# maelaubert/VulkanSift

Hardware: AMD Instinct MI355X
Metric: SIFT detect+match frames/sec (640x480, ~2k kp) (higher is better)
Workload: dtype f32

## Files before the change

include/vksift_hip.h:

```cpp
#ifndef VKSIFT_HIP_H
#define VKSIFT_HIP_H

#include <stddef.h>
#include <stdint.h>

#ifdef __cplusplus
extern "C"
{
#endif

#define VKSIFT_HIP_MAX_TAPS 20
#define VKSIFT_HIP_MATCH_CHUNKS 32
#define VKSIFT_HIP_MATCH_SMALL_NA 1536u
#define VKSIFT_HIP_MATCH_SMALL_NB 4096u
#define VKSIFT_HIP_MATCH_SCRATCH_U32(na, nb) (2u * (size_t)(na) + (size_t)(nb) + 72u + (size_t)(na) * 16u * VKSIFT_HIP_MATCH_CHUNKS)
#define VKSIFT_HIP_ABI_VERSION 6u
#define VKSIFT_HIP_GATHER_SLOTS 512u
#define VKSIFT_HIP_MATCH_SLOTS 256u
#define VKSIFT_HIP_MATCH_PK_NB 32768u
#define VKSIFT_HIP_MAX_ORI 18
#define VKSIFT_HIP_MAX_OCTAVE_SIDE 16383u

  typedef void *vksift_hip_stream;
  typedef void *vksift_hip_graph;
// ... 22 lines not shown
  int vksift_hip_event_sync(vksift_hip_event e);
  int vksift_hip_event_busy(vksift_hip_event e);
  float vksift_hip_event_elapsed_ms(vksift_hip_event a, vksift_hip_event b);
  int vksift_hip_stream_wait_event(vksift_hip_stream s, vksift_hip_event e);
  int vksift_hip_capture_begin(vksift_hip_stream s);
  int vksift_hip_capture_end(vksift_hip_stream s, vksift_hip_graph *out);
  int vksift_hip_graph_launch(vksift_hip_graph g, vksift_hip_stream s);
  void vksift_hip_graph_destroy(vksift_hip_graph g);
  int vksift_hip_memcpy_h2d(void *dst, const void *src, size_t n, vksift_hip_stream s);
  int vksift_hip_memcpy_d2h(void *dst, const void *src, size_t n, vksift_hip_stream s);
  int vksift_hip_memcpy_d2d(void *dst, const void *src, size_t n, vksift_hip_stream s);
  int vksift_hip_memcpy2d_d2h(void *dst, size_t dpitch, const void *src, size_t spitch, size_t width_bytes, size_t height, vksift_hip_stream s);
  int vksift_hip_post_words(uint32_t *host_mapped_dst, const uint32_t *src, size_t n_words, vksift_hip_stream s);
  int vksift_hip_memset(void *dst, int value, size_t n, vksift_hip_stream s);
  const char *vksift_hip_error_string(int err);
  void vksift_hip_range_push(const char *name);
  void vksift_hip_range_pop(void);

  enum
  {
    VKSIFT_TUNE_WG_TARGET = 0,
    VKSIFT_TUNE_WIDE_MASK = 1,
    VKSIFT_TUNE_MULTI_MAX = 2,
    VKSIFT_TUNE_REFINE_PTR = 3,
    VKSIFT_TUNE_SCAN_FORM = 4,
    VKSIFT_TUNE_PAIR_FORM = 5,
    VKSIFT_TUNE_PYR_GATE = 6,
    VKSIFT_TUNE_DENSE_ROWS = 7,
    VKSIFT_TUNE_SEED_WG = 8,
    VKSIFT_TUNE_SCAN_BAND = 9,
    VKSIFT_TUNE_TAIL_MULTI = 10,
    VKSIFT_TUNE_ZERO_COPY = 11,
    VKSIFT_TUNE_MIN_MARCH = 12,
    VKSIFT_TUNE_COUNT = 16
  };
  int vksift_hip_tune(int knob, int value);
  int vksift_hip_tune_get(int knob);


  typedef struct
  {
    float *base;
    uint32_t w, h;
    uint32_t pitch;
    uint64_t img_stride;
    uint32_t fp16;
    uint32_t reverse;
  } vksift_hip_Plane;

  int vksift_hip_input_blit(const uint8_t *src, uint32_t sw, uint32_t sh, uint64_t src_img_stride, vksift_hip_Plane dst, uint32_t batch,
                            vksift_hip_stream s);

  int vksift_hip_blur(vksift_hip_Plane src, vksift_hip_Plane dst, const float *taps, uint32_t ntaps, uint32_t batch, vksift_hip_stream s);

  int vksift_hip_blur_pair(vksift_hip_Plane src, vksift_hip_Plane dst1, vksift_hip_Plane dst2, const float *taps1, uint32_t ntaps1, const float *taps2,
                           uint32_t ntaps2, uint32_t batch, vksift_hip_stream s);

  int vksift_hip_blur_form(vksift_hip_Plane src, vksift_hip_Plane dst, uint32_t ntaps, uint32_t batch);

  int vksift_hip_blur_multi(const vksift_hip_Plane *src, const vksift_hip_Plane *dst, uint32_t n, const float *taps, uint32_t ntaps, uint32_t batch,
                            vksift_hip_stream s);

  int vksift_hip_blur_downsample(vksift_hip_Plane src, vksift_hip_Plane dst, vksift_hip_Plane next, const float *taps, uint32_t ntaps, uint32_t batch,
                                 vksift_hip_stream s);

  int vksift_hip_seed_upsampled(const uint8_t *src, uint32_t sw, uint32_t sh, uint64_t src_img_stride, vksift_hip_Plane dst, const float *taps, uint32_t ntaps,
// ... 133 lines not shown
```

vulkansift_amd/build.py:

```python
import hashlib
import os
import subprocess
import sys

PKG = os.path.dirname(os.path.abspath(__file__))
ROOT = os.path.dirname(PKG)
CSRC = os.path.join(PKG, "csrc")
OUT_DIR = os.path.join(PKG, "lib")
OBJ_DIR = os.path.join(OUT_DIR, "obj")
LIB_PATH = os.path.join(OUT_DIR, "libvulkansift.so")

HOST_SRCS = ["host/vksift_api.c", "host/vksift_instance.c", "host/vksift_mem.c", "host/vksift_detect.c", "host/vksift_stage.c", "host/vksift_defer.c", "host/vksift_buffers.c", "host/vksift_match.c", "host/vksift_verify.c", "host/vksift_refine.c", "host/vksift_guided.c",
             "host/vksift_ext.c", "host/vksift_sharded.c", "host/vksift_hostmath.c", "host/vksift_log.c", "host/vksift_synth.c"]
HIP_SRCS = ["hip/runtime.hip", "hip/pyramid.hip", "hip/extrema.hip", "hip/features.hip", "hip/match.hip", "hip/records.hip", "hip/verify.hip", "hip/refine.hip", "hip/refine_f.hip", "hip/guided.hip"]

ROCM = os.environ.get("ROCM_PATH", "/opt/rocm")
HIPCC = os.path.join(ROCM, "bin", "hipcc")
INCLUDES = ["-I" + os.path.join(ROOT, "include"), "-I" + os.path.join(CSRC, "host"), "-I" + CSRC]

CFLAGS = ["-O2", "-std=gnu11", "-fPIC", "-fexceptions", "-ffp-contract=off", "-fno-fast-math", "-mavx2", "-mfma", "-Wall", "-Wextra",
          "-Wno-unused-parameter"]
HIPFLAGS = ["--offload-arch=gfx950", "-O3", "-std=c++17", "-fPIC", "-ffp-contract=off", "-fno-fast-math", "-Wall", "-Wno-unused-function",
            "-fno-gpu-rdc"]


def _newer(target, deps):
    if not os.path.exists(target):
        return True
    t = os.path.getmtime(target)
    return any(os.path.getmtime(d) > t for d in deps if os.path.exists(d))


_TOOL_VERSION = {}


def _tool_version(tool):
    if tool not in _TOOL_VERSION:
        r = subprocess.run([tool, "--version"], capture_output=True, text=True)
        _TOOL_VERSION[tool] = (r.stdout + r.stderr).strip()
    return _TOOL_VERSION[tool]


def _signature(cmd, src, headers):
    h = hashlib.sha256()
    h.update(("\0".join(cmd).replace(ROOT, "<root>") + "\0" + _tool_version(cmd[0])).encode())
    for path in [src] + sorted(headers):
        h.update(os.path.relpath(path, ROOT).encode() + b"\0")
# ... 97 lines not shown
```

vulkansift_amd/csrc/hip/extrema.hip:

```cpp
#include <hip/hip_runtime.h>
#include <type_traits>
#include <vector>
#include <stdint.h>
#include <stdlib.h>

#include "../detmath.h"
#include "multi.h"
#include "records.h"
#include "vksift_hip.h"

namespace
{

struct DogView
{
  const float *base;
  int w, h, pitch;
  size_t plane;
  int S;
};

template <bool F16>
__device__ __forceinline__ float ld(const DogView &d, int s, int x, int y)
{
  if (s < 0 || s > d.S + 1)
    return 0.f;
  if (F16)
  {
    const _Float16 *p = (const _Float16 *)d.base + (size_t)s * d.plane + (size_t)y * d.pitch + x;
    return (float)(_Float16)((float)p[d.plane] - (float)p[0]);
  }
  const float *p = d.base + (size_t)s * d.plane + (size_t)y * d.pitch + x;
  return p[d.plane] - p[0];
}

struct KpRecord
{
  float x, y, scale_x, scale_y;
  uint32_t scale_idx;
  int32_t octave_idx;
  float sigma, orientation, intensity;
};

struct Dog19
{
  float c;
  float sp, sm, xp, xm, yp, ym;
  float sp_xp, sp_xm, sm_xp, sm_xm;
  float sp_yp, sp_ym, sm_yp, sm_ym;
  float xp_yp, xp_ym, xm_yp, xm_ym;
};

template <bool F16>
struct PtrLoader
{
  static constexpr int UNROLL_STEPS = 1;
  const DogView &d;
  __device__ __forceinline__ Dog19 operator()(int x, int y, int s) const
  {
    Dog19 v;
    v.c = ld<F16>(d, s, x, y);
    v.sp = ld<F16>(d, s + 1, x, y), v.sm = ld<F16>(d, s - 1, x, y);
    v.xp = ld<F16>(d, s, x + 1, y), v.xm = ld<F16>(d, s, x - 1, y);
    v.yp = ld<F16>(d, s, x, y + 1), v.ym = ld<F16>(d, s, x, y - 1);
    v.sp_xp = ld<F16>(d, s + 1, x + 1, y), v.sp_xm = ld<F16>(d, s + 1, x - 1, y), v.sm_xp = ld<F16>(d, s - 1, x + 1, y), v.sm_xm = ld<F16>(d, s - 1, x - 1, y);
    v.sp_yp = ld<F16>(d, s + 1, x, y + 1), v.sp_ym = ld<F16>(d, s + 1, x, y - 1), v.sm_yp = ld<F16>(d, s - 1, x, y + 1), v.sm_ym = ld<F16>(d, s - 1, x, y - 1);
    v.xp_yp = ld<F16>(d, s, x + 1, y + 1), v.xp_ym = ld<F16>(d, s, x + 1, y - 1), v.xm_yp = ld<F16>(d, s, x - 1, y + 1), v.xm_ym = ld<F16>(d, s, x - 1, y - 1);
    return v;
  }
};

template <bool F16>
struct BufLoader
{
  static constexpr int UNROLL_STEPS = 5;
  static constexpr unsigned EB = F16 ? 2u : 4u;
  const __amdgpu_buffer_rsrc_t rsrc;
  const int pitch;
  const unsigned plane;
  const int S;
  __device__ __forceinline__ float tex(unsigned base, int row_off) const
  {
    if (F16)
      return (float)__builtin_bit_cast(_Float16, (unsigned short)__builtin_amdgcn_raw_buffer_load_b16(rsrc, base, row_off, 0));
    return __uint_as_float(__builtin_amdgcn_raw_buffer_load_b32(rsrc, base, row_off, 0));
  }
  static __device__ __forceinline__ float dog(float hi, float lo) { return F16 ? (float)(_Float16)(hi - lo) : hi - lo; }
  __device__ __forceinline__ Dog19 operator()(int x, int y, int s) const
  {
    const int pitch_b = pitch * (int)EB;
    const unsigned plane_b = plane * EB;
    const unsigned b0 = ((unsigned)s * plane + (unsigned)(y - 1) * (unsigned)pitch + (unsigned)(x - 1)) * EB;
    const unsigned bm = b0 - plane_b, b1 = b0 + plane_b, b2 = b1 + plane_b;
    float g0[3][3], g1[3][3];
#pragma unroll
    for (int j = 0; j < 3; j++)
#pragma unroll
      for (int i = 0; i < 3; i++)
      {
        g0[j][i] = tex(b0 + (unsigned)i * EB, j * pitch_b);
        g1[j][i] = tex(b1 + (unsigned)i * EB, j * pitch_b);
      }
    const float gm_c = tex(bm + EB, pitch_b), gm_xm = tex(bm, pitch_b), gm_xp = tex(bm + 2u * EB, pitch_b), gm_ym = tex(bm + EB, 0), gm_yp = tex(bm + EB, 2 * pitch_b);
    const float g2_c = tex(b2 + EB, pitch_b), g2_xm = tex(b2, pitch_b), g2_xp = tex(b2 + 2u * EB, pitch_b), g2_ym = tex(b2 + EB, 0), g2_yp = tex(b2 + EB, 2 * pitch_b);
    const bool up = s + 1 <= S + 1;
    Dog19 v;
    v.sp = up ? dog(g2_c, g1[1][1]) : 0.f, v.sm = dog(g0[1][1], gm_c);
    v.sp_xp = up ? dog(g2_xp, g1[1][2]) : 0.f, v.sp_xm = up ? dog(g2_xm, g1[1][0]) : 0.f;
    v.sp_yp = up ? dog(g2_yp, g1[2][1]) : 0.f, v.sp_ym = up ? dog(g2_ym, g1[0][1]) : 0.f;
    v.sm_xp = dog(g0[1][2], gm_xp), v.sm_xm = dog(g0[1][0], gm_xm), v.sm_yp = dog(g0[2][1], gm_yp), v.sm_ym = dog(g0[0][1], gm_ym);
    float d0[3][3];
#pragma unroll
    for (int j = 0; j < 3; j++)
#pragma unroll
      for (int i = 0; i < 3; i++)
        d0[j][i] = dog(g1[j][i], g0[j][i]);
    v.c = d0[1][1];
    v.xp = d0[1][2], v.xm = d0[1][0], v.yp = d0[2][1], v.ym = d0[0][1];
    v.xp_yp = d0[2][2], v.xp_ym = d0[0][2], v.xm_yp = d0[2][0], v.xm_ym = d0[0][0];
    return v;
  }
};

template <class Load>
__device__ bool refine_core(const Load &load, int W, int H, int S, int x, int y, int s, float dog_threshold, float edge_limit, float seed_sigma, int octave_idx,
                            KpRecord *kp)
{
  float oX = 0.f, oY = 0.f, oS = 0.f, gX = 0.f, gY = 0.f, gS = 0.f;
  float vc = 0.f, xp = 0.f, xm = 0.f, yp = 0.f, ym = 0.f, h23 = 0.f;
  int rx = x, ry = y, rs = s;
#pragma unroll Load::UNROLL_STEPS
  for (int step = 0; step < 5; step++)
  {
    const Dog19 v = load(rx, ry, rs);
    vc = v.c;
    xp = v.xp, xm = v.xm, yp = v.yp, ym = v.ym;
    gS = 0.5f * (v.sp - v.sm);
    gX = 0.5f * (xp - xm);
    gY = 0.5f * (yp - ym);
    float h11 = v.sp + v.sm - 2.f * vc;
    float h22 = xp + xm - 2.f * vc;
    float h33 = yp + ym - 2.f * vc;
    float h12 = 0.25f * (v.sp_xp - v.sp_xm - v.sm_xp + v.sm_xm);
    float h13 = 0.25f * (v.sp_yp - v.sp_ym - v.sm_yp + v.sm_ym);
    h23 = 0.25f * (v.xp_yp - v.xp_ym - v.xm_yp + v.xm_ym);

    float det = h11 * ((h22 * h33) - (h23 * h23)) - h12 * ((h12 * h33) - (h13 * h23)) + h13 * ((h12 * h23) - (h13 * h22));
    if (det == 0.0f)
      return false;
    float i11 = ((h22 * h33) - (h23 * h23)) / det;
    float i12 = -1.f * ((h12 * h33) - (h13 * h23)) / det;
    float i13 = ((h12 * h23) - (h13 * h22)) / det;
    float i22 = ((h11 * h33) - (h13 * h13)) / det;
    float i23 = -1.f * ((h11 * h23) - (h13 * h12)) / det;
    float i33 = ((h11 * h22) - (h12 * h12)) / det;
    oS = -i11 * gS - i12 * gX - i13 * gY;
    oX = -i12 * gS - i22 * gX - i23 * gY;
    oY = -i13 * gS - i23 * gX - i33 * gY;

    if (fabsf(oX) < 0.6f && fabsf(oY) < 0.6f && fabsf(oS) < 0.6f)
      break;
    else if (step < 4)
    {
      rx += ((oX >= 0.6f && rx < (W - 2)) ? 1 : 0) + ((oX <= -0.6f && rx > 1) ? -1 : 0);
      ry += ((oY >= 0.6f && ry < (H - 2)) ? 1 : 0) + ((oY <= -0.6f && ry > 1) ? -1 : 0);
      rs += ((oS >= 0.6f && rs < (S + 1)) ? 1 : 0) + ((oS <= -0.6f && rs > 1) ? -1 : 0);
    }
  }
  float sx = (float)rx + oX, sy = (float)ry + oY, ss = (float)rs + oS;
  float nv = vc + 0.5f * (gX * oX + gY * oY + gS * oS);
  if (!(fabsf(nv) > dog_threshold && fabsf(oX) < 1.5f && fabsf(oY) < 1.5f && fabsf(oS) < 1.5f && sx >= 0 && sx < (float)W && sy >= 0 && sy < (float)H &&
        ss >= 0 && ss <= (float)(S + 1)))
    return false;
  float e11 = xp + xm - 2.f * vc;
  float e22 = yp + ym - 2.f * vc;
  float e12 = h23;
  float edgeness = ((e11 + e22) * (e11 + e22)) / ((e11 * e22) - (e12 * e12));
  if (!((edgeness < edge_limit) && (edgeness >= 0)))
    return false;

  float scale_factor = octave_idx >= 0 ? dm_pow2i(octave_idx) : 1.f / dm_pow2i(-octave_idx);
  kp->scale_x = sx;
  kp->scale_y = sy;
  kp->scale_idx = (uint32_t)roundf(ss);
  kp->octave_idx = octave_idx;
  kp->sigma = seed_sigma * dm_exp2f(ss / (float)S) * scale_factor;
  kp->orientation = 0.f;
  kp->intensity = nv;
  kp->x = sx * scale_factor;
  kp->y = sy * scale_factor;
  return true;
}

__device__ __forceinline__ void store_record(uint32_t *rec, const KpRecord &kp)
{
  static_assert(sizeof(KpRecord) == VKSIFT_RECORD_HEAD_WORDS * 4u, "the header words of a stored record");
  rec[0] = __float_as_uint(kp.x);
  rec[1] = __float_as_uint(kp.y);
  rec[2] = __float_as_uint(kp.scale_x);
  rec[3] = __float_as_uint(kp.scale_y);
  rec[4] = kp.scale_idx;
  rec[5] = (uint32_t)kp.octave_idx;
  rec[6] = __float_as_uint(kp.sigma);
  rec[7] = __float_as_uint(kp.orientation);
  rec[8] = __float_as_uint(kp.intensity);
}

struct ExtremaArgs
{
  const float *gauss;
  int fp16;
  int w, h, pitch;
  uint64_t plane_stride, img_stride;
  int S, octave_idx;
  float seed_sigma, dog_threshold, edge_limit;
  uint64_t *seg_mask;
  uint32_t *seg_off;
  uint64_t seg_img_stride;
  int nseg;
  uint8_t *feats;
  uint64_t feat_img_stride;
  uint32_t cap;
  uint32_t *found;
  uint32_t found_img_stride;
  uint32_t *cand_xy;
  uint32_t *cand_flag;
  uint32_t *cand_n;
  uint64_t cand_img_stride;
  uint32_t cand_cap;
  int band;
  uint32_t nsegs;
  uint32_t nchunks;
  int scan_rev;
};

__device__ __forceinline__ float wave_shr1(float v, float edge)
{
  return __builtin_bit_cast(float, __builtin_amdgcn_update_dpp(__builtin_bit_cast(int, edge), __builtin_bit_cast(int, v), 0x138, 0xf, 0xf, false));
}
__device__ __forceinline__ float wave_shl1(float v, float edge)
{
  return __builtin_bit_cast(float, __builtin_amdgcn_update_dpp(__builtin_bit_cast(int, edge), __builtin_bit_cast(int, v), 0x130, 0xf, 0xf, false));
}

__device__ __forceinline__ float fmax2(float a, float b)
{
  float r;
  asm("v_max_f32 %0, %1, %2" : "=v"(r) : "v"(a), "v"(b));
  return r;
}
__device__ __forceinline__ float fmin2(float a, float b)
{
  float r;
  asm("v_min_f32 %0, %1, %2" : "=v"(r) : "v"(a), "v"(b));
  return r;
}
__device__ __forceinline__ float fmax3(float a, float b, float c)
{
  float r;
  asm("v_max3_f32 %0, %1, %2, %3" : "=v"(r) : "v"(a), "v"(b), "v"(c));
  return r;
}
__device__ __forceinline__ float fmin3(float a, float b, float c)
{
  float r;
  asm("v_min3_f32 %0, %1, %2, %3" : "=v"(r) : "v"(a), "v"(b), "v"(c));
  return r;
}

__device__ __forceinline__ uint32_t wave_sum_u32(uint32_t v)
{
#pragma unroll
  for (int dlt = 32; dlt >= 1; dlt >>= 1)
    v += __shfl_xor(v, dlt, 64);
  return v;
}

__device__ __forceinline__ unsigned long long spread32(unsigned long long x)
{
  x &= 0xFFFFFFFFull;
  x = (x | (x << 16)) & 0x0000FFFF0000FFFFull;
  x = (x | (x << 8)) & 0x00FF00FF00FF00FFull;
  x = (x | (x << 4)) & 0x0F0F0F0F0F0F0F0Full;
  x = (x | (x << 2)) & 0x3333333333333333ull;
  x = (x | (x << 1)) & 0x5555555555555555ull;
  return x;
}

typedef unsigned u32x2_t __attribute__((ext_vector_type(2)));
constexpr unsigned EXT_OOB = 0x80000000u;

template <int S, int NSLOT, bool F16>
__global__ void __launch_bounds__(256, 4) k_extrema_lean(Multi<ExtremaArgs> m, int strip_major)
{
  const VBlock vb = vblock(m);
  const ExtremaArgs &a = m.oct[vb.o];
  const int band = a.band;
  constexpr int NL = S + 2;
  constexpr int EB = F16 ? 2 : 4;
  constexpr int AHEAD = NSLOT - 3;
  const int lane = threadIdx.x & 63;
  const int wv = __builtin_amdgcn_readfirstlane((int)(threadIdx.x >> 6));
  int b = vb.z;
  int bx = vb.x, by = vb.y * 4 + wv;
  if (strip_major)
  {
    unsigned blk = vb.y * vb.gx + vb.x;
    if (strip_major & 2)
// ... 225 lines not shown
  const int b = (int)vb.y;
  const uint32_t *chunk_tot = a.cand_flag + (size_t)b * a.cand_img_stride;
  if (vb.x == 0 && threadIdx.x == 0)
  {
    uint32_t total = 0;
    for (uint32_t c = 0; c < a.nchunks; c++)
      total += chunk_tot[c];
    a.cand_n[b] = total;
    if (total == 0)
      a.found[(size_t)b * a.found_img_stride] = 0;
  }
  unsigned long long m = seg < a.nsegs ? a.seg_mask[seg + (size_t)b * a.seg_img_stride] : 0ull;
  if (__ballot(m != 0ull) == 0ull)
    return;
  uint32_t base = 0;
  for (uint32_t c = threadIdx.x & 63u, nc = (vb.x * 256u) / SEG_CHUNK; c < nc; c += 64u)
    base += chunk_tot[c];
  base = wave_sum_u32(base);
  if (m == 0ull)
    return;
  uint32_t pos = a.seg_off[seg + (size_t)b * a.seg_img_stride] + base;
  const uint32_t segx = seg % (uint32_t)a.nseg;
  const uint32_t yy = (seg / (uint32_t)a.nseg) % (uint32_t)a.h;
  const uint32_t sz = seg / ((uint32_t)a.nseg * (uint32_t)a.h);
  uint32_t *out = a.cand_xy + (size_t)b * a.cand_img_stride;
  while (m)
  {
    const int bit = __ffsll((long long)m) - 1;
    m &= m - 1;
    if (pos < a.cand_cap)
      out[pos] = (segx * 64u + (uint32_t)bit) | (yy << 14) | ((sz + 1u) << 28);
    pos++;
  }
}

struct RefineCtx
{
  const ExtremaArgs &a;
  uint32_t n, nch;
  DogView d;
  __amdgpu_buffer_rsrc_t rsrc;
  const uint32_t *xy;
  uint32_t *flag, *chunk_sum;
};

template <bool F16>
__device__ __forceinline__ RefineCtx refine_ctx(const ExtremaArgs &a, int b)
{
  constexpr unsigned EB = F16 ? 2u : 4u;
  const uint32_t found = a.cand_n[b], n = found < a.cand_cap ? found : a.cand_cap;
  const DogView d{(const float *)((const uint8_t *)a.gauss + (size_t)b * a.img_stride * EB), a.w, a.h, a.pitch, (size_t)a.plane_stride, a.S};
  const __amdgpu_buffer_rsrc_t rsrc = __builtin_amdgcn_make_buffer_rsrc((void *)d.base, 0, (int)((unsigned)(a.S + 3) * (unsigned)a.plane_stride * EB), 0x00020000);
  const size_t at = (size_t)b * a.cand_img_stride;
  return RefineCtx{a, n, (n + 255u) / 256u, d, rsrc, a.cand_xy + at, a.cand_flag + at, a.seg_off + (size_t)b * a.seg_img_stride};
}

template <bool F16, bool BUF>
__device__ __forceinline__ bool refine_candidate(const RefineCtx &c, uint32_t packed, KpRecord *kp)
{
  const ExtremaArgs &a = c.a;
  const int x = (int)(packed & 0x3fffu), y = (int)((packed >> 14) & 0x3fffu), s = (int)(packed >> 28);
  if constexpr (BUF)
    return refine_core(BufLoader<F16>{c.rsrc, a.pitch, (unsigned)a.plane_stride, a.S}, a.w, a.h, a.S, x, y, s, a.dog_threshold, a.edge_limit, a.seed_sigma, a.octave_idx, kp);
  else
    return refine_core(PtrLoader<F16>{c.d}, a.w, a.h, a.S, x, y, s, a.dog_threshold, a.edge_limit, a.seed_sigma, a.octave_idx, kp);
}

template <bool F16, bool BUF>
__global__ void __launch_bounds__(256) k_refine_flags(Multi<ExtremaArgs> m)
{
  __shared__ uint32_t s_cnt[4];
  const VBlock vb = vblock(m);
  const RefineCtx c = refine_ctx<F16>(m.oct[vb.o], (int)vb.x);
  for (uint32_t chunk = vb.y; chunk < c.nch; chunk += vb.gy)
  {
    const uint32_t i = chunk * 256u + threadIdx.x;
    bool ok = false;
    if (i < c.n)
    {
      KpRecord kp;
      ok = refine_candidate<F16, BUF>(c, c.xy[i], &kp);
      c.flag[i] = ok ? 1u : 0u;
    }
    const unsigned long long bal = __ballot(ok);
    if ((threadIdx.x & 63) == 0)
      s_cnt[threadIdx.x >> 6] = (uint32_t)__popcll(bal);
    __syncthreads();
    if (threadIdx.x == 0)
      c.chunk_sum[chunk] = s_cnt[0] + s_cnt[1] + s_cnt[2] + s_cnt[3];
    __syncthreads();
  }
}

template <bool F16, bool BUF>
__global__ void __launch_bounds__(256) k_cand_emit(Multi<ExtremaArgs> m)
{
  __shared__ uint32_t s_cnt[4];
  __shared__ uint32_t s_red[4];
// ... 106 lines not shown
    cleared = cleared && jobs[i].masks_cleared != 0;
  if (!cleared)
  {
    const int me = clear_masks(args, n, batch, hs);
    if (me)
      return me;
  }
  const int sm = 3;

#define VKSIFT_MULTI(M, GX, GY, GZ)                              \
  Multi<ExtremaArgs> M;                                           \
  M.n = 0;                                                        \
  for (uint32_t i = 0; i < n; i++)                                \
  {                                                               \
    const ExtremaArgs &a = args[i];                               \
    (void)a;                                                      \
    if (!multi_add(M, args[i], (GX), (GY), (GZ)))                 \
      return (int)hipErrorInvalidValue;                           \
  }
  {
    VKSIFT_MULTI(ms, (uint32_t)(a.nseg + 1) / 2u, ((a.h + a.band - 1) / a.band + 3u) / 4u, batch)
    const dim3 sgrid(ms.start[ms.n]);
    const bool known = with_scales(S, [&](auto NS) {
      with_bool(f16, [&](auto F16) {
        constexpr bool h = decltype(F16)::value;
        hipLaunchKernelGGL((k_extrema_lean<decltype(NS)::value, h ? 5 : 4, h>), sgrid, dim3(256), 0, hs, ms, sm);
      });
    });
    if (!known)
      return (int)hipErrorInvalidValue;
  }
  if (scan_done)
    (void)hipEventRecord(scan_done, hs);
  {
    VKSIFT_MULTI(m2, a.nchunks, batch, 1u)
    hipLaunchKernelGGL(k_segment_scan, dim3(m2.start[m2.n]), dim3(1024), 0, hs, m2);
  }
  {
    VKSIFT_MULTI(m3, (a.nsegs + 255u) / 256u, batch, 1u)
    hipLaunchKernelGGL(k_cand_list, dim3(m3.start[m3.n]), dim3(256), 0, hs, m3);
  }
  const uint32_t rcap = 65536u / batch < 16u ? 16u : (65536u / batch > 512u ? 512u : 65536u / batch);
#define VKSIFT_REFINE_CHUNKS(a) (((uint64_t)(a).S * (uint32_t)(a).w * (uint32_t)(a).h / 4u + 64u + 255u) / 256u)
  VKSIFT_MULTI(mr, batch, VKSIFT_REFINE_CHUNKS(a) > rcap ? rcap : (uint32_t)VKSIFT_REFINE_CHUNKS(a), 1u)
#undef VKSIFT_REFINE_CHUNKS
#undef VKSIFT_MULTI
  const dim3 rgrid(mr.start[mr.n]);
  bool buf = vksift_hip_tune_get(VKSIFT_TUNE_REFINE_PTR) == 0;
  for (uint32_t i = 0; i < n; i++)
    buf = buf && (uint64_t)(args[i].S + 3) * args[i].plane_stride * (f16 ? 2u : 4u) < 0x7FFF0000ull;
  with_bool(f16, [&](auto F16) {
    with_bool(buf, [&](auto BUF) {
      hipLaunchKernelGGL((k_refine_flags<decltype(F16)::value, decltype(BUF)::value>), rgrid, dim3(256), 0, hs, mr);
      hipLaunchKernelGGL((k_cand_emit<decltype(F16)::value, decltype(BUF)::value>), rgrid, dim3(256), 0, hs, mr);
    });
  });
  return (int)hipGetLastError();
}

static int make_all_extrema_args(const vksift_hip_OctaveJob *jobs, uint32_t n_jobs, std::vector<ExtremaArgs> &args)
{
  args.resize(n_jobs);
  for (uint32_t i = 0; i < n_jobs; i++)
  {
    const int e = make_extrema_args(&jobs[i], &args[i]);
    if (e)
      return e;
  }
  return 0;
}

extern "C" int vksift_hip_extract_keypoints_multi(const vksift_hip_OctaveJob *jobs, uint32_t n_jobs, uint32_t batch, vksift_hip_stream s,
                                                  vksift_hip_event scan_done)
{
  if (n_jobs == 0 || batch == 0)
    return 0;
  std::vector<ExtremaArgs> args;
  const int bad = make_all_extrema_args(jobs, n_jobs, args);
  if (bad)
    return bad;
  for (uint32_t i0 = 0; i0 < n_jobs;)
  {
    uint32_t i1 = i0 + 1;
// ... 26 lines not shown
```

Measured before the change: 25180.

## Fuse segment scan, candidate listing and refinement into one tail kernel

```diff
diff --git a/include/vksift_hip.h b/include/vksift_hip.h
--- a/include/vksift_hip.h
+++ b/include/vksift_hip.h
@@ -78,6 +78,7 @@
     VKSIFT_TUNE_TAIL_MULTI = 10,
     VKSIFT_TUNE_ZERO_COPY = 11,
     VKSIFT_TUNE_MIN_MARCH = 12,
+    VKSIFT_TUNE_TAIL_FUSED = 13,
     VKSIFT_TUNE_COUNT = 16
   };
   int vksift_hip_tune(int knob, int value);
diff --git a/vulkansift_amd/build.py b/vulkansift_amd/build.py
--- a/vulkansift_amd/build.py
+++ b/vulkansift_amd/build.py
@@ -12,7 +12,7 @@
 
 HOST_SRCS = ["host/vksift_api.c", "host/vksift_instance.c", "host/vksift_mem.c", "host/vksift_detect.c", "host/vksift_stage.c", "host/vksift_defer.c", "host/vksift_buffers.c", "host/vksift_match.c", "host/vksift_verify.c", "host/vksift_refine.c", "host/vksift_guided.c",
              "host/vksift_ext.c", "host/vksift_sharded.c", "host/vksift_hostmath.c", "host/vksift_log.c", "host/vksift_synth.c"]
-HIP_SRCS = ["hip/runtime.hip", "hip/pyramid.hip", "hip/extrema.hip", "hip/features.hip", "hip/match.hip", "hip/records.hip", "hip/verify.hip", "hip/refine.hip", "hip/refine_f.hip", "hip/guided.hip"]
+HIP_SRCS = ["hip/runtime.hip", "hip/pyramid.hip", "hip/extrema.hip", "hip/extract_tail.hip", "hip/features.hip", "hip/match.hip", "hip/records.hip", "hip/verify.hip", "hip/refine.hip", "hip/refine_f.hip", "hip/guided.hip"]
 
 ROCM = os.environ.get("ROCM_PATH", "/opt/rocm")
 HIPCC = os.path.join(ROCM, "bin", "hipcc")
diff --git a/vulkansift_amd/csrc/hip/extract_tail.hip b/vulkansift_amd/csrc/hip/extract_tail.hip
--- /dev/null
+++ b/vulkansift_amd/csrc/hip/extract_tail.hip
@@ -0,0 +1,161 @@
+#include <hip/hip_runtime.h>
+#include <stdint.h>
+
+#include "extrema_refine.h"
+#include "multi.h"
+#include "records.h"
+#include "vksift_hip.h"
+
+namespace
+{
+
+constexpr uint32_t TAIL_SPT = 2;
+constexpr uint32_t TAIL_LIST = 4096;
+
+template <bool F16, bool BUF>
+__global__ void __launch_bounds__(1024) __attribute__((amdgpu_waves_per_eu(6, 8))) k_extract_tail(Multi<ExtremaArgs> m)
+{
+  __shared__ uint32_t s_list[TAIL_LIST];
+  __shared__ uint32_t s_wtot[2][16];
+  __shared__ uint32_t s_cnt[2][16];
+  const VBlock vb = vblock(m);
+  const ExtremaArgs &a = m.oct[vb.o];
+  const int b = (int)vb.x;
+  const uint32_t tid = threadIdx.x, NT = blockDim.x, nw = NT >> 6, lane = tid & 63u, wave = tid >> 6;
+  constexpr unsigned EB = F16 ? 2u : 4u;
+  const DogView d{(const float *)((const uint8_t *)a.gauss + (size_t)b * a.img_stride * EB), a.w, a.h, a.pitch, (size_t)a.plane_stride, a.S};
+  const __amdgpu_buffer_rsrc_t rsrc = __builtin_amdgcn_make_buffer_rsrc((void *)d.base, 0, (int)((unsigned)(a.S + 3) * (unsigned)a.plane_stride * EB), 0x00020000);
+  const RefineCtx c{a, 0u, 0u, d, rsrc, nullptr, nullptr, nullptr};
+  const uint64_t *__restrict__ mask = a.seg_mask + (size_t)b * a.seg_img_stride;
+  uint8_t *const feats = a.feats + (size_t)b * a.feat_img_stride;
+  const uint32_t nsegs = a.nsegs, tile = NT * TAIL_SPT;
+
+  uint32_t base = 0;
+  uint32_t ncand = 0;
+  uint32_t fill = 0;
+  uint32_t rpar = 0;
+
+  auto round = [&](uint32_t c0, uint32_t cnt) {
+    KpRecord kp;
+    bool ok = false;
+    if (tid < cnt)
+      ok = refine_candidate<F16, BUF>(c, s_list[c0 + tid], &kp);
+    const unsigned long long bal = __ballot(ok);
+    if (lane == 0)
+      s_cnt[rpar][wave] = (uint32_t)__popcll(bal);
+    __syncthreads();
+    uint32_t rank = (uint32_t)__popcll(bal & ((1ull << lane) - 1ull)), total = 0;
+    for (uint32_t wv = 0; wv < nw; wv++)
+    {
+      const uint32_t n = s_cnt[rpar][wv];
+      rank += wv < wave ? n : 0u;
+      total += n;
+    }
+    const uint32_t idx = base + rank;
+    if (ok && idx < a.cap)
+      store_record((uint32_t *)(feats + (size_t)idx * VKSIFT_RECORD_BYTES), kp);
+    base += total;
+    rpar ^= 1u;
+  };
+
+  auto load_tile = [&](uint32_t t0, unsigned long long(&mk)[TAIL_SPT]) {
+    const uint32_t i0 = t0 + TAIL_SPT * tid;
+#pragma unroll
+    for (uint32_t k = 0; k < TAIL_SPT; k++)
+      mk[k] = i0 + k < nsegs ? mask[i0 + k] : 0ull;
+  };
+
+  unsigned long long cur[TAIL_SPT];
+  uint32_t tpar = 0;
+  for (uint32_t t0 = 0; t0 < nsegs; t0 += tile, tpar ^= 1u)
+  {
+    load_tile(t0, cur);
+    uint32_t tsum = 0;
+#pragma unroll
+    for (uint32_t k = 0; k < TAIL_SPT; k++)
+      tsum += (uint32_t)__popcll(cur[k]);
+    uint32_t incl = tsum;
+#pragma unroll
+    for (int dlt = 1; dlt < 64; dlt <<= 1)
+    {
+      const uint32_t t = __shfl_up(incl, dlt, 64);
+      if ((int)lane >= dlt)
+        incl += t;
+    }
+    if (lane == 63u)
+      s_wtot[tpar][wave] = incl;
+    __syncthreads();
+    uint32_t off = incl - tsum, T = 0;
+    for (uint32_t wv = 0; wv < nw; wv++)
+    {
+      const uint32_t n = s_wtot[tpar][wv];
+      off += wv < wave ? n : 0u;
+      T += n;
+    }
+    const uint32_t valid = ncand >= a.cand_cap ? 0u : (T < a.cand_cap - ncand ? T : a.cand_cap - ncand);
+    ncand += T;
+    for (uint32_t w0 = 0; w0 < valid;)
+    {
+      const uint32_t room = TAIL_LIST - fill, hi = valid - w0 < room ? valid : w0 + room;
+      if (off < hi && off + tsum > w0)
+      {
+        uint32_t pos = off;
+#pragma unroll
+        for (uint32_t k = 0; k < TAIL_SPT; k++)
+        {
+          unsigned long long mk = cur[k];
+          if (mk == 0ull)
+            continue;
+          const uint32_t seg = t0 + TAIL_SPT * tid + k;
+          const uint32_t row = seg / (uint32_t)a.nseg, segx = seg - row * (uint32_t)a.nseg;
+          const uint32_t sz = row / (uint32_t)a.h, yy = row - sz * (uint32_t)a.h;
+          const uint32_t head = (segx * 64u) | (yy << 14) | ((sz + 1u) << 28);
+          while (mk)
+          {
+            const uint32_t bit = (uint32_t)__ffsll((long long)mk) - 1u;
+            mk &= mk - 1ull;
+            if (pos >= w0 && pos < hi)
+              s_list[fill + (pos - w0)] = head + bit;
+            pos++;
+          }
+        }
+      }
+      fill += hi - w0;
+      w0 = hi;
+      __syncthreads();
+      const uint32_t nfull = fill - fill % NT, left = fill - nfull;
+      for (uint32_t c0 = 0; c0 < nfull; c0 += NT)
+        round(c0, NT);
+      if (nfull != 0u && left != 0u)
+      {
+        if (tid < left)
+          s_list[tid] = s_list[nfull + tid];
+        __syncthreads();
+      }
+      fill = left;
+    }
+  }
+  if (fill != 0u)
+    round(0u, fill);
+  if (tid == 0u)
+  {
+    a.cand_n[b] = ncand;
+    a.found[(size_t)b * a.found_img_stride] = base;
+  }
+}
+
+}
+
+int extract_tail_launch(const ExtremaArgs *args, uint32_t n, uint32_t batch, bool f16, bool buf, bool small_wg, hipStream_t hs)
+{
+  Multi<ExtremaArgs> mt;
+  mt.n = 0;
+  for (uint32_t i = 0; i < n; i++)
+    if (!multi_add(mt, args[i], batch, 1u, 1u))
+      return (int)hipErrorInvalidValue;
+  const dim3 grid(mt.start[mt.n]), block(mt.start[mt.n] < 512u && !small_wg ? 1024u : 512u);
+  with_bool(f16, [&](auto F16) {
+    with_bool(buf, [&](auto BUF) { hipLaunchKernelGGL((k_extract_tail<decltype(F16)::value, decltype(BUF)::value>), grid, block, 0, hs, mt); });
+  });
+  return (int)hipGetLastError();
+}
diff --git a/vulkansift_amd/csrc/hip/extrema.hip b/vulkansift_amd/csrc/hip/extrema.hip
--- a/vulkansift_amd/csrc/hip/extrema.hip
+++ b/vulkansift_amd/csrc/hip/extrema.hip
@@ -5,6 +5,7 @@
 #include <stdlib.h>
 
 #include "../detmath.h"
+#include "extrema_refine.h"
 #include "multi.h"
 #include "records.h"
 #include "vksift_hip.h"
@@ -12,228 +13,6 @@
 namespace
 {
 
-struct DogView
-{
-  const float *base;
-  int w, h, pitch;
-  size_t plane;
-  int S;
-};
-
-template <bool F16>
-__device__ __forceinline__ float ld(const DogView &d, int s, int x, int y)
-{
-  if (s < 0 || s > d.S + 1)
-    return 0.f;
-  if (F16)
-  {
-    const _Float16 *p = (const _Float16 *)d.base + (size_t)s * d.plane + (size_t)y * d.pitch + x;
-    return (float)(_Float16)((float)p[d.plane] - (float)p[0]);
-  }
-  const float *p = d.base + (size_t)s * d.plane + (size_t)y * d.pitch + x;
-  return p[d.plane] - p[0];
-}
-
-struct KpRecord
-{
-  float x, y, scale_x, scale_y;
-  uint32_t scale_idx;
-  int32_t octave_idx;
-  float sigma, orientation, intensity;
-};
-
-struct Dog19
-{
-  float c;
-  float sp, sm, xp, xm, yp, ym;
-  float sp_xp, sp_xm, sm_xp, sm_xm;
-  float sp_yp, sp_ym, sm_yp, sm_ym;
-  float xp_yp, xp_ym, xm_yp, xm_ym;
-};
-
-template <bool F16>
-struct PtrLoader
-{
-  static constexpr int UNROLL_STEPS = 1;
-  const DogView &d;
-  __device__ __forceinline__ Dog19 operator()(int x, int y, int s) const
-  {
-    Dog19 v;
-    v.c = ld<F16>(d, s, x, y);
-    v.sp = ld<F16>(d, s + 1, x, y), v.sm = ld<F16>(d, s - 1, x, y);
-    v.xp = ld<F16>(d, s, x + 1, y), v.xm = ld<F16>(d, s, x - 1, y);
-    v.yp = ld<F16>(d, s, x, y + 1), v.ym = ld<F16>(d, s, x, y - 1);
-    v.sp_xp = ld<F16>(d, s + 1, x + 1, y), v.sp_xm = ld<F16>(d, s + 1, x - 1, y), v.sm_xp = ld<F16>(d, s - 1, x + 1, y), v.sm_xm = ld<F16>(d, s - 1, x - 1, y);
-    v.sp_yp = ld<F16>(d, s + 1, x, y + 1), v.sp_ym = ld<F16>(d, s + 1, x, y - 1), v.sm_yp = ld<F16>(d, s - 1, x, y + 1), v.sm_ym = ld<F16>(d, s - 1, x, y - 1);
-    v.xp_yp = ld<F16>(d, s, x + 1, y + 1), v.xp_ym = ld<F16>(d, s, x + 1, y - 1), v.xm_yp = ld<F16>(d, s, x - 1, y + 1), v.xm_ym = ld<F16>(d, s, x - 1, y - 1);
-    return v;
-  }
-};
-
-template <bool F16>
-struct BufLoader
-{
-  static constexpr int UNROLL_STEPS = 5;
-  static constexpr unsigned EB = F16 ? 2u : 4u;
-  const __amdgpu_buffer_rsrc_t rsrc;
-  const int pitch;
-  const unsigned plane;
-  const int S;
-  __device__ __forceinline__ float tex(unsigned base, int row_off) const
-  {
-    if (F16)
-      return (float)__builtin_bit_cast(_Float16, (unsigned short)__builtin_amdgcn_raw_buffer_load_b16(rsrc, base, row_off, 0));
-    return __uint_as_float(__builtin_amdgcn_raw_buffer_load_b32(rsrc, base, row_off, 0));
-  }
-  static __device__ __forceinline__ float dog(float hi, float lo) { return F16 ? (float)(_Float16)(hi - lo) : hi - lo; }
-  __device__ __forceinline__ Dog19 operator()(int x, int y, int s) const
-  {
-    const int pitch_b = pitch * (int)EB;
-    const unsigned plane_b = plane * EB;
-    const unsigned b0 = ((unsigned)s * plane + (unsigned)(y - 1) * (unsigned)pitch + (unsigned)(x - 1)) * EB;
-    const unsigned bm = b0 - plane_b, b1 = b0 + plane_b, b2 = b1 + plane_b;
-    float g0[3][3], g1[3][3];
-#pragma unroll
-    for (int j = 0; j < 3; j++)
-#pragma unroll
-      for (int i = 0; i < 3; i++)
-      {
-        g0[j][i] = tex(b0 + (unsigned)i * EB, j * pitch_b);
-        g1[j][i] = tex(b1 + (unsigned)i * EB, j * pitch_b);
-      }
-    const float gm_c = tex(bm + EB, pitch_b), gm_xm = tex(bm, pitch_b), gm_xp = tex(bm + 2u * EB, pitch_b), gm_ym = tex(bm + EB, 0), gm_yp = tex(bm + EB, 2 * pitch_b);
-    const float g2_c = tex(b2 + EB, pitch_b), g2_xm = tex(b2, pitch_b), g2_xp = tex(b2 + 2u * EB, pitch_b), g2_ym = tex(b2 + EB, 0), g2_yp = tex(b2 + EB, 2 * pitch_b);
-    const bool up = s + 1 <= S + 1;
-    Dog19 v;
-    v.sp = up ? dog(g2_c, g1[1][1]) : 0.f, v.sm = dog(g0[1][1], gm_c);
-    v.sp_xp = up ? dog(g2_xp, g1[1][2]) : 0.f, v.sp_xm = up ? dog(g2_xm, g1[1][0]) : 0.f;
-    v.sp_yp = up ? dog(g2_yp, g1[2][1]) : 0.f, v.sp_ym = up ? dog(g2_ym, g1[0][1]) : 0.f;
-    v.sm_xp = dog(g0[1][2], gm_xp), v.sm_xm = dog(g0[1][0], gm_xm), v.sm_yp = dog(g0[2][1], gm_yp), v.sm_ym = dog(g0[0][1], gm_ym);
-    float d0[3][3];
-#pragma unroll
-    for (int j = 0; j < 3; j++)
-#pragma unroll
-      for (int i = 0; i < 3; i++)
-        d0[j][i] = dog(g1[j][i], g0[j][i]);
-    v.c = d0[1][1];
-    v.xp = d0[1][2], v.xm = d0[1][0], v.yp = d0[2][1], v.ym = d0[0][1];
-    v.xp_yp = d0[2][2], v.xp_ym = d0[0][2], v.xm_yp = d0[2][0], v.xm_ym = d0[0][0];
-    return v;
-  }
-};
-
-template <class Load>
-__device__ bool refine_core(const Load &load, int W, int H, int S, int x, int y, int s, float dog_threshold, float edge_limit, float seed_sigma, int octave_idx,
-                            KpRecord *kp)
-{
-  float oX = 0.f, oY = 0.f, oS = 0.f, gX = 0.f, gY = 0.f, gS = 0.f;
-  float vc = 0.f, xp = 0.f, xm = 0.f, yp = 0.f, ym = 0.f, h23 = 0.f;
-  int rx = x, ry = y, rs = s;
-#pragma unroll Load::UNROLL_STEPS
-  for (int step = 0; step < 5; step++)
-  {
-    const Dog19 v = load(rx, ry, rs);
-    vc = v.c;
-    xp = v.xp, xm = v.xm, yp = v.yp, ym = v.ym;
-    gS = 0.5f * (v.sp - v.sm);
-    gX = 0.5f * (xp - xm);
-    gY = 0.5f * (yp - ym);
-    float h11 = v.sp + v.sm - 2.f * vc;
-    float h22 = xp + xm - 2.f * vc;
-    float h33 = yp + ym - 2.f * vc;
-    float h12 = 0.25f * (v.sp_xp - v.sp_xm - v.sm_xp + v.sm_xm);
-    float h13 = 0.25f * (v.sp_yp - v.sp_ym - v.sm_yp + v.sm_ym);
-    h23 = 0.25f * (v.xp_yp - v.xp_ym - v.xm_yp + v.xm_ym);
-
-    float det = h11 * ((h22 * h33) - (h23 * h23)) - h12 * ((h12 * h33) - (h13 * h23)) + h13 * ((h12 * h23) - (h13 * h22));
-    if (det == 0.0f)
-      return false;
-    float i11 = ((h22 * h33) - (h23 * h23)) / det;
-    float i12 = -1.f * ((h12 * h33) - (h13 * h23)) / det;
-    float i13 = ((h12 * h23) - (h13 * h22)) / det;
-    float i22 = ((h11 * h33) - (h13 * h13)) / det;
-    float i23 = -1.f * ((h11 * h23) - (h13 * h12)) / det;
-    float i33 = ((h11 * h22) - (h12 * h12)) / det;
-    oS = -i11 * gS - i12 * gX - i13 * gY;
-    oX = -i12 * gS - i22 * gX - i23 * gY;
-    oY = -i13 * gS - i23 * gX - i33 * gY;
-
-    if (fabsf(oX) < 0.6f && fabsf(oY) < 0.6f && fabsf(oS) < 0.6f)
-      break;
-    else if (step < 4)
-    {
-      rx += ((oX >= 0.6f && rx < (W - 2)) ? 1 : 0) + ((oX <= -0.6f && rx > 1) ? -1 : 0);
-      ry += ((oY >= 0.6f && ry < (H - 2)) ? 1 : 0) + ((oY <= -0.6f && ry > 1) ? -1 : 0);
-      rs += ((oS >= 0.6f && rs < (S + 1)) ? 1 : 0) + ((oS <= -0.6f && rs > 1) ? -1 : 0);
-    }
-  }
-  float sx = (float)rx + oX, sy = (float)ry + oY, ss = (float)rs + oS;
-  float nv = vc + 0.5f * (gX * oX + gY * oY + gS * oS);
-  if (!(fabsf(nv) > dog_threshold && fabsf(oX) < 1.5f && fabsf(oY) < 1.5f && fabsf(oS) < 1.5f && sx >= 0 && sx < (float)W && sy >= 0 && sy < (float)H &&
-        ss >= 0 && ss <= (float)(S + 1)))
-    return false;
-  float e11 = xp + xm - 2.f * vc;
-  float e22 = yp + ym - 2.f * vc;
-  float e12 = h23;
-  float edgeness = ((e11 + e22) * (e11 + e22)) / ((e11 * e22) - (e12 * e12));
-  if (!((edgeness < edge_limit) && (edgeness >= 0)))
-    return false;
-
-  float scale_factor = octave_idx >= 0 ? dm_pow2i(octave_idx) : 1.f / dm_pow2i(-octave_idx);
-  kp->scale_x = sx;
-  kp->scale_y = sy;
-  kp->scale_idx = (uint32_t)roundf(ss);
-  kp->octave_idx = octave_idx;
-  kp->sigma = seed_sigma * dm_exp2f(ss / (float)S) * scale_factor;
-  kp->orientation = 0.f;
-  kp->intensity = nv;
-  kp->x = sx * scale_factor;
-  kp->y = sy * scale_factor;
-  return true;
-}
-
-__device__ __forceinline__ void store_record(uint32_t *rec, const KpRecord &kp)
-{
-  static_assert(sizeof(KpRecord) == VKSIFT_RECORD_HEAD_WORDS * 4u, "the header words of a stored record");
-  rec[0] = __float_as_uint(kp.x);
-  rec[1] = __float_as_uint(kp.y);
-  rec[2] = __float_as_uint(kp.scale_x);
-  rec[3] = __float_as_uint(kp.scale_y);
-  rec[4] = kp.scale_idx;
-  rec[5] = (uint32_t)kp.octave_idx;
-  rec[6] = __float_as_uint(kp.sigma);
-  rec[7] = __float_as_uint(kp.orientation);
-  rec[8] = __float_as_uint(kp.intensity);
-}
-
-struct ExtremaArgs
-{
-  const float *gauss;
-  int fp16;
-  int w, h, pitch;
-  uint64_t plane_stride, img_stride;
-  int S, octave_idx;
-  float seed_sigma, dog_threshold, edge_limit;
-  uint64_t *seg_mask;
-  uint32_t *seg_off;
-  uint64_t seg_img_stride;
-  int nseg;
-  uint8_t *feats;
-  uint64_t feat_img_stride;
-  uint32_t cap;
-  uint32_t *found;
-  uint32_t found_img_stride;
-  uint32_t *cand_xy;
-  uint32_t *cand_flag;
-  uint32_t *cand_n;
-  uint64_t cand_img_stride;
-  uint32_t cand_cap;
-  int band;
-  uint32_t nsegs;
-  uint32_t nchunks;
-  int scan_rev;
-};
-
 __device__ __forceinline__ float wave_shr1(float v, float edge)
 {
   return __builtin_bit_cast(float, __builtin_amdgcn_update_dpp(__builtin_bit_cast(int, edge), __builtin_bit_cast(int, v), 0x138, 0xf, 0xf, false));
@@ -266,14 +45,6 @@
   float r;
   asm("v_min3_f32 %0, %1, %2, %3" : "=v"(r) : "v"(a), "v"(b), "v"(c));
   return r;
-}
-
-__device__ __forceinline__ uint32_t wave_sum_u32(uint32_t v)
-{
-#pragma unroll
-  for (int dlt = 32; dlt >= 1; dlt >>= 1)
-    v += __shfl_xor(v, dlt, 64);
-  return v;
 }
 
 __device__ __forceinline__ unsigned long long spread32(unsigned long long x)
@@ -565,38 +336,6 @@
       out[pos] = (segx * 64u + (uint32_t)bit) | (yy << 14) | ((sz + 1u) << 28);
     pos++;
   }
-}
-
-struct RefineCtx
-{
-  const ExtremaArgs &a;
-  uint32_t n, nch;
-  DogView d;
-  __amdgpu_buffer_rsrc_t rsrc;
-  const uint32_t *xy;
-  uint32_t *flag, *chunk_sum;
-};
-
-template <bool F16>
-__device__ __forceinline__ RefineCtx refine_ctx(const ExtremaArgs &a, int b)
-{
-  constexpr unsigned EB = F16 ? 2u : 4u;
-  const uint32_t found = a.cand_n[b], n = found < a.cand_cap ? found : a.cand_cap;
-  const DogView d{(const float *)((const uint8_t *)a.gauss + (size_t)b * a.img_stride * EB), a.w, a.h, a.pitch, (size_t)a.plane_stride, a.S};
-  const __amdgpu_buffer_rsrc_t rsrc = __builtin_amdgcn_make_buffer_rsrc((void *)d.base, 0, (int)((unsigned)(a.S + 3) * (unsigned)a.plane_stride * EB), 0x00020000);
-  const size_t at = (size_t)b * a.cand_img_stride;
-  return RefineCtx{a, n, (n + 255u) / 256u, d, rsrc, a.cand_xy + at, a.cand_flag + at, a.seg_off + (size_t)b * a.seg_img_stride};
-}
-
-template <bool F16, bool BUF>
-__device__ __forceinline__ bool refine_candidate(const RefineCtx &c, uint32_t packed, KpRecord *kp)
-{
-  const ExtremaArgs &a = c.a;
-  const int x = (int)(packed & 0x3fffu), y = (int)((packed >> 14) & 0x3fffu), s = (int)(packed >> 28);
-  if constexpr (BUF)
-    return refine_core(BufLoader<F16>{c.rsrc, a.pitch, (unsigned)a.plane_stride, a.S}, a.w, a.h, a.S, x, y, s, a.dog_threshold, a.edge_limit, a.seed_sigma, a.octave_idx, kp);
-  else
-    return refine_core(PtrLoader<F16>{c.d}, a.w, a.h, a.S, x, y, s, a.dog_threshold, a.edge_limit, a.seed_sigma, a.octave_idx, kp);
 }
 
 template <bool F16, bool BUF>
@@ -769,6 +508,12 @@
   }
   if (scan_done)
     (void)hipEventRecord(scan_done, hs);
+  bool buf = vksift_hip_tune_get(VKSIFT_TUNE_REFINE_PTR) == 0;
+  for (uint32_t i = 0; i < n; i++)
+    buf = buf && (uint64_t)(args[i].S + 3) * args[i].plane_stride * (f16 ? 2u : 4u) < 0x7FFF0000ull;
+  const int fused = vksift_hip_tune_get(VKSIFT_TUNE_TAIL_FUSED);
+  if (fused == 2 || fused == 3 || (fused != 1 && batch >= 64u))
+    return extract_tail_launch(args, n, batch, f16, buf, fused == 3, hs);
   {
     VKSIFT_MULTI(m2, a.nchunks, batch, 1u)
     hipLaunchKernelGGL(k_segment_scan, dim3(m2.start[m2.n]), dim3(1024), 0, hs, m2);
@@ -783,9 +528,6 @@
 #undef VKSIFT_REFINE_CHUNKS
 #undef VKSIFT_MULTI
   const dim3 rgrid(mr.start[mr.n]);
-  bool buf = vksift_hip_tune_get(VKSIFT_TUNE_REFINE_PTR) == 0;
-  for (uint32_t i = 0; i < n; i++)
-    buf = buf && (uint64_t)(args[i].S + 3) * args[i].plane_stride * (f16 ? 2u : 4u) < 0x7FFF0000ull;
   with_bool(f16, [&](auto F16) {
     with_bool(buf, [&](auto BUF) {
       hipLaunchKernelGGL((k_refine_flags<decltype(F16)::value, decltype(BUF)::value>), rgrid, dim3(256), 0, hs, mr);
diff --git a/vulkansift_amd/csrc/hip/extrema_refine.h b/vulkansift_amd/csrc/hip/extrema_refine.h
--- /dev/null
+++ b/vulkansift_amd/csrc/hip/extrema_refine.h
@@ -0,0 +1,276 @@
+#pragma once
+#include <hip/hip_runtime.h>
+#include <stdint.h>
+
+#include "../detmath.h"
+#include "records.h"
+#include "vksift_hip.h"
+
+struct ExtremaArgs
+{
+  const float *gauss;
+  int fp16;
+  int w, h, pitch;
+  uint64_t plane_stride, img_stride;
+  int S, octave_idx;
+  float seed_sigma, dog_threshold, edge_limit;
+  uint64_t *seg_mask;
+  uint32_t *seg_off;
+  uint64_t seg_img_stride;
+  int nseg;
+  uint8_t *feats;
+  uint64_t feat_img_stride;
+  uint32_t cap;
+  uint32_t *found;
+  uint32_t found_img_stride;
+  uint32_t *cand_xy;
+  uint32_t *cand_flag;
+  uint32_t *cand_n;
+  uint64_t cand_img_stride;
+  uint32_t cand_cap;
+  int band;
+  uint32_t nsegs;
+  uint32_t nchunks;
+  int scan_rev;
+};
+
+namespace
+{
+
+struct DogView
+{
+  const float *base;
+  int w, h, pitch;
+  size_t plane;
+  int S;
+};
+
+template <bool F16>
+__device__ __forceinline__ float ld(const DogView &d, int s, int x, int y)
+{
+  if (s < 0 || s > d.S + 1)
+    return 0.f;
+  if (F16)
+  {
+    const _Float16 *p = (const _Float16 *)d.base + (size_t)s * d.plane + (size_t)y * d.pitch + x;
+    return (float)(_Float16)((float)p[d.plane] - (float)p[0]);
+  }
+  const float *p = d.base + (size_t)s * d.plane + (size_t)y * d.pitch + x;
+  return p[d.plane] - p[0];
+}
+
+struct KpRecord
+{
+  float x, y, scale_x, scale_y;
+  uint32_t scale_idx;
+  int32_t octave_idx;
+  float sigma, orientation, intensity;
+};
+
+struct Dog19
+{
+  float c;
+  float sp, sm, xp, xm, yp, ym;
+  float sp_xp, sp_xm, sm_xp, sm_xm;
+  float sp_yp, sp_ym, sm_yp, sm_ym;
+  float xp_yp, xp_ym, xm_yp, xm_ym;
+};
+
+template <bool F16>
+struct PtrLoader
+{
+  static constexpr int UNROLL_STEPS = 1;
+  const DogView &d;
+  __device__ __forceinline__ Dog19 operator()(int x, int y, int s) const
+  {
+    Dog19 v;
+    v.c = ld<F16>(d, s, x, y);
+    v.sp = ld<F16>(d, s + 1, x, y), v.sm = ld<F16>(d, s - 1, x, y);
+    v.xp = ld<F16>(d, s, x + 1, y), v.xm = ld<F16>(d, s, x - 1, y);
+    v.yp = ld<F16>(d, s, x, y + 1), v.ym = ld<F16>(d, s, x, y - 1);
+    v.sp_xp = ld<F16>(d, s + 1, x + 1, y), v.sp_xm = ld<F16>(d, s + 1, x - 1, y), v.sm_xp = ld<F16>(d, s - 1, x + 1, y), v.sm_xm = ld<F16>(d, s - 1, x - 1, y);
+    v.sp_yp = ld<F16>(d, s + 1, x, y + 1), v.sp_ym = ld<F16>(d, s + 1, x, y - 1), v.sm_yp = ld<F16>(d, s - 1, x, y + 1), v.sm_ym = ld<F16>(d, s - 1, x, y - 1);
+    v.xp_yp = ld<F16>(d, s, x + 1, y + 1), v.xp_ym = ld<F16>(d, s, x + 1, y - 1), v.xm_yp = ld<F16>(d, s, x - 1, y + 1), v.xm_ym = ld<F16>(d, s, x - 1, y - 1);
+    return v;
+  }
+};
+
+template <bool F16>
+struct BufLoader
+{
+  static constexpr int UNROLL_STEPS = 5;
+  static constexpr unsigned EB = F16 ? 2u : 4u;
+  const __amdgpu_buffer_rsrc_t rsrc;
+  const int pitch;
+  const unsigned plane;
+  const int S;
+  __device__ __forceinline__ float tex(unsigned base, int row_off) const
+  {
+    if (F16)
+      return (float)__builtin_bit_cast(_Float16, (unsigned short)__builtin_amdgcn_raw_buffer_load_b16(rsrc, base, row_off, 0));
+    return __uint_as_float(__builtin_amdgcn_raw_buffer_load_b32(rsrc, base, row_off, 0));
+  }
+  static __device__ __forceinline__ float dog(float hi, float lo) { return F16 ? (float)(_Float16)(hi - lo) : hi - lo; }
+  __device__ __forceinline__ Dog19 operator()(int x, int y, int s) const
+  {
+    const int pitch_b = pitch * (int)EB;
+    const unsigned plane_b = plane * EB;
+    const unsigned b0 = ((unsigned)s * plane + (unsigned)(y - 1) * (unsigned)pitch + (unsigned)(x - 1)) * EB;
+    const unsigned bm = b0 - plane_b, b1 = b0 + plane_b, b2 = b1 + plane_b;
+    float g0[3][3], g1[3][3];
+#pragma unroll
+    for (int j = 0; j < 3; j++)
+#pragma unroll
+      for (int i = 0; i < 3; i++)
+      {
+        g0[j][i] = tex(b0 + (unsigned)i * EB, j * pitch_b);
+        g1[j][i] = tex(b1 + (unsigned)i * EB, j * pitch_b);
+      }
+    const float gm_c = tex(bm + EB, pitch_b), gm_xm = tex(bm, pitch_b), gm_xp = tex(bm + 2u * EB, pitch_b), gm_ym = tex(bm + EB, 0), gm_yp = tex(bm + EB, 2 * pitch_b);
+    const float g2_c = tex(b2 + EB, pitch_b), g2_xm = tex(b2, pitch_b), g2_xp = tex(b2 + 2u * EB, pitch_b), g2_ym = tex(b2 + EB, 0), g2_yp = tex(b2 + EB, 2 * pitch_b);
+    const bool up = s + 1 <= S + 1;
+    Dog19 v;
+    v.sp = up ? dog(g2_c, g1[1][1]) : 0.f, v.sm = dog(g0[1][1], gm_c);
+    v.sp_xp = up ? dog(g2_xp, g1[1][2]) : 0.f, v.sp_xm = up ? dog(g2_xm, g1[1][0]) : 0.f;
+    v.sp_yp = up ? dog(g2_yp, g1[2][1]) : 0.f, v.sp_ym = up ? dog(g2_ym, g1[0][1]) : 0.f;
+    v.sm_xp = dog(g0[1][2], gm_xp), v.sm_xm = dog(g0[1][0], gm_xm), v.sm_yp = dog(g0[2][1], gm_yp), v.sm_ym = dog(g0[0][1], gm_ym);
+    float d0[3][3];
+#pragma unroll
+    for (int j = 0; j < 3; j++)
+#pragma unroll
+      for (int i = 0; i < 3; i++)
+        d0[j][i] = dog(g1[j][i], g0[j][i]);
+    v.c = d0[1][1];
+    v.xp = d0[1][2], v.xm = d0[1][0], v.yp = d0[2][1], v.ym = d0[0][1];
+    v.xp_yp = d0[2][2], v.xp_ym = d0[0][2], v.xm_yp = d0[2][0], v.xm_ym = d0[0][0];
+    return v;
+  }
+};
+
+template <class Load>
+__device__ bool refine_core(const Load &load, int W, int H, int S, int x, int y, int s, float dog_threshold, float edge_limit, float seed_sigma, int octave_idx,
+                            KpRecord *kp)
+{
+  float oX = 0.f, oY = 0.f, oS = 0.f, gX = 0.f, gY = 0.f, gS = 0.f;
+  float vc = 0.f, xp = 0.f, xm = 0.f, yp = 0.f, ym = 0.f, h23 = 0.f;
+  int rx = x, ry = y, rs = s;
+#pragma unroll Load::UNROLL_STEPS
+  for (int step = 0; step < 5; step++)
+  {
+    const Dog19 v = load(rx, ry, rs);
+    vc = v.c;
+    xp = v.xp, xm = v.xm, yp = v.yp, ym = v.ym;
+    gS = 0.5f * (v.sp - v.sm);
+    gX = 0.5f * (xp - xm);
+    gY = 0.5f * (yp - ym);
+    float h11 = v.sp + v.sm - 2.f * vc;
+    float h22 = xp + xm - 2.f * vc;
+    float h33 = yp + ym - 2.f * vc;
+    float h12 = 0.25f * (v.sp_xp - v.sp_xm - v.sm_xp + v.sm_xm);
+    float h13 = 0.25f * (v.sp_yp - v.sp_ym - v.sm_yp + v.sm_ym);
+    h23 = 0.25f * (v.xp_yp - v.xp_ym - v.xm_yp + v.xm_ym);
+
+    float det = h11 * ((h22 * h33) - (h23 * h23)) - h12 * ((h12 * h33) - (h13 * h23)) + h13 * ((h12 * h23) - (h13 * h22));
+    if (det == 0.0f)
+      return false;
+    float i11 = ((h22 * h33) - (h23 * h23)) / det;
+    float i12 = -1.f * ((h12 * h33) - (h13 * h23)) / det;
+    float i13 = ((h12 * h23) - (h13 * h22)) / det;
+    float i22 = ((h11 * h33) - (h13 * h13)) / det;
+    float i23 = -1.f * ((h11 * h23) - (h13 * h12)) / det;
+    float i33 = ((h11 * h22) - (h12 * h12)) / det;
+    oS = -i11 * gS - i12 * gX - i13 * gY;
+    oX = -i12 * gS - i22 * gX - i23 * gY;
+    oY = -i13 * gS - i23 * gX - i33 * gY;
+
+    if (fabsf(oX) < 0.6f && fabsf(oY) < 0.6f && fabsf(oS) < 0.6f)
+      break;
+    else if (step < 4)
+    {
+      rx += ((oX >= 0.6f && rx < (W - 2)) ? 1 : 0) + ((oX <= -0.6f && rx > 1) ? -1 : 0);
+      ry += ((oY >= 0.6f && ry < (H - 2)) ? 1 : 0) + ((oY <= -0.6f && ry > 1) ? -1 : 0);
+      rs += ((oS >= 0.6f && rs < (S + 1)) ? 1 : 0) + ((oS <= -0.6f && rs > 1) ? -1 : 0);
+    }
+  }
+  float sx = (float)rx + oX, sy = (float)ry + oY, ss = (float)rs + oS;
+  float nv = vc + 0.5f * (gX * oX + gY * oY + gS * oS);
+  if (!(fabsf(nv) > dog_threshold && fabsf(oX) < 1.5f && fabsf(oY) < 1.5f && fabsf(oS) < 1.5f && sx >= 0 && sx < (float)W && sy >= 0 && sy < (float)H &&
+        ss >= 0 && ss <= (float)(S + 1)))
+    return false;
+  float e11 = xp + xm - 2.f * vc;
+  float e22 = yp + ym - 2.f * vc;
+  float e12 = h23;
+  float edgeness = ((e11 + e22) * (e11 + e22)) / ((e11 * e22) - (e12 * e12));
+  if (!((edgeness < edge_limit) && (edgeness >= 0)))
+    return false;
+
+  float scale_factor = octave_idx >= 0 ? dm_pow2i(octave_idx) : 1.f / dm_pow2i(-octave_idx);
+  kp->scale_x = sx;
+  kp->scale_y = sy;
+  kp->scale_idx = (uint32_t)roundf(ss);
+  kp->octave_idx = octave_idx;
+  kp->sigma = seed_sigma * dm_exp2f(ss / (float)S) * scale_factor;
+  kp->orientation = 0.f;
+  kp->intensity = nv;
+  kp->x = sx * scale_factor;
+  kp->y = sy * scale_factor;
+  return true;
+}
+
+__device__ __forceinline__ void store_record(uint32_t *rec, const KpRecord &kp)
+{
+  static_assert(sizeof(KpRecord) == VKSIFT_RECORD_HEAD_WORDS * 4u, "the header words of a stored record");
+  rec[0] = __float_as_uint(kp.x);
+  rec[1] = __float_as_uint(kp.y);
+  rec[2] = __float_as_uint(kp.scale_x);
+  rec[3] = __float_as_uint(kp.scale_y);
+  rec[4] = kp.scale_idx;
+  rec[5] = (uint32_t)kp.octave_idx;
+  rec[6] = __float_as_uint(kp.sigma);
+  rec[7] = __float_as_uint(kp.orientation);
+  rec[8] = __float_as_uint(kp.intensity);
+}
+
+__device__ __forceinline__ uint32_t wave_sum_u32(uint32_t v)
+{
+#pragma unroll
+  for (int dlt = 32; dlt >= 1; dlt >>= 1)
+    v += __shfl_xor(v, dlt, 64);
+  return v;
+}
+
+struct RefineCtx
+{
+  const ExtremaArgs &a;
+  uint32_t n, nch;
+  DogView d;
+  __amdgpu_buffer_rsrc_t rsrc;
+  const uint32_t *xy;
+  uint32_t *flag, *chunk_sum;
+};
+
+template <bool F16>
+__device__ __forceinline__ RefineCtx refine_ctx(const ExtremaArgs &a, int b)
+{
+  constexpr unsigned EB = F16 ? 2u : 4u;
+  const uint32_t found = a.cand_n[b], n = found < a.cand_cap ? found : a.cand_cap;
+  const DogView d{(const float *)((const uint8_t *)a.gauss + (size_t)b * a.img_stride * EB), a.w, a.h, a.pitch, (size_t)a.plane_stride, a.S};
+  const __amdgpu_buffer_rsrc_t rsrc = __builtin_amdgcn_make_buffer_rsrc((void *)d.base, 0, (int)((unsigned)(a.S + 3) * (unsigned)a.plane_stride * EB), 0x00020000);
+  const size_t at = (size_t)b * a.cand_img_stride;
+  return RefineCtx{a, n, (n + 255u) / 256u, d, rsrc, a.cand_xy + at, a.cand_flag + at, a.seg_off + (size_t)b * a.seg_img_stride};
+}
+
+template <bool F16, bool BUF>
+__device__ __forceinline__ bool refine_candidate(const RefineCtx &c, uint32_t packed, KpRecord *kp)
+{
+  const ExtremaArgs &a = c.a;
+  const int x = (int)(packed & 0x3fffu), y = (int)((packed >> 14) & 0x3fffu), s = (int)(packed >> 28);
+  if constexpr (BUF)
+    return refine_core(BufLoader<F16>{c.rsrc, a.pitch, (unsigned)a.plane_stride, a.S}, a.w, a.h, a.S, x, y, s, a.dog_threshold, a.edge_limit, a.seed_sigma, a.octave_idx, kp);
+  else
+    return refine_core(PtrLoader<F16>{c.d}, a.w, a.h, a.S, x, y, s, a.dog_threshold, a.edge_limit, a.seed_sigma, a.octave_idx, kp);
+}
+
+}
+
+int extract_tail_launch(const ExtremaArgs *args, uint32_t n, uint32_t batch, bool f16, bool buf, bool small_wg, hipStream_t hs);
```

Result: faster. 25710, median of 6 (+2.1%).
